# sadit/Jchemo.jl

Measured on AMD Instinct MI355X. Metric: latent-variables/sec (plskern n=1e6 p=500 q=10 nlv=25), higher is better.
Workload: dtype f64

## Files before the change

### jchemo.jl_amd/csrc/bf16.hip

```cpp
#include <stdlib.h>

#include <algorithm>
#include <type_traits>

#include "jch_internal.h"

typedef double v4f64 __attribute__((ext_vector_type(4)));
typedef unsigned short bf16_t;
typedef unsigned int v4u32 __attribute__((ext_vector_type(4)));

__device__ __forceinline__ float bf2f(bf16_t h) { return __uint_as_float(((unsigned)h) << 16); }
__device__ __forceinline__ float bflo(unsigned w) { return __uint_as_float(w << 16); }
__device__ __forceinline__ float bfhi(unsigned w) { return __uint_as_float(w & 0xffff0000u); }

template <bool VAR>
__global__ __launch_bounds__(256) void k_moments_bf16(const bf16_t *__restrict__ Xc, int64_t ldx, const bf16_t *__restrict__ Yc,
                                                       int64_t ldy, const double *__restrict__ d, int64_t n, int p, int q,
                                                       int64_t chunk, const double *__restrict__ means,
                                                       double *__restrict__ colpart)
{
    __shared__ double sc[4];
    const int j = blockIdx.x;
    const bf16_t *col = j < p ? Xc + (size_t)j * (size_t)ldx : Yc + (size_t)(j - p) * (size_t)ldy;
    const int64_t i0 = (int64_t)blockIdx.y * chunk;
// ... 594 lines not shown
        for (; b < nbx; b += 4) s0 += Kpart[(size_t)b * stride + e];
    }
    sc[g][el] = (s0 + s1) + (s2 + s3);
    __syncthreads();
    if (g == 0 && e < p * qpad) K[e] = (sc[0][el] + sc[1][el]) + (sc[2][el] + sc[3][el]);
}

template <int R>
__device__ __forceinline__ void wave_sum_rows(float (&s)[R], float (&t)[R])
{
    static_assert(R == 2 || R == 4 || R == 8, "R");
    const int lane = threadIdx.x & 63;
    float cur[R];
#pragma unroll
    for (int i = 0; i < R; ++i) cur[i] = s[i];
    int width = R;
    int bit = 32;
#pragma unroll
    for (int st = 0; st < 3; ++st) {
        if (width > 1) {
            const int half = width / 2;
            const bool hi = (lane & bit) != 0;
#pragma unroll
            for (int i = 0; i < R / 2; ++i) {
                if (i < half) {
                    const float mine = hi ? cur[half + i] : cur[i];
                    const float other = hi ? cur[i] : cur[half + i];
                    cur[i] = mine + __shfl_xor(other, bit, 64);
                }
            }
            width = half;
            bit >>= 1;
        }
    }
    float c = cur[0];
    for (int o = bit; o > 0; o >>= 1) c += __shfl_xor(c, o, 64);
#pragma unroll
    for (int r = 0; r < R; ++r) {
        int src = 0;
        if (R == 8) src = ((r >> 2) & 1) * 32 + ((r >> 1) & 1) * 16 + (r & 1) * 8;
        if (R == 4) src = ((r >> 1) & 1) * 32 + (r & 1) * 16;
        if (R == 2) src = (r & 1) * 32;
        t[r] = __int_as_float(__builtin_amdgcn_readlane(__float_as_int(c), src));
    }
}

template <int KC, int R>
__global__ __launch_bounds__(256) void k_sweep_bf16(const bf16_t *__restrict__ Xr, int64_t n, int ldr, const double *__restrict__ dw,
                                                    const double *__restrict__ rvec, const double *__restrict__ mom,
                                                    const double *__restrict__ scl, int p,
                                                    double *__restrict__ tcol, double *__restrict__ part, int ldpart)
{
    extern __shared__ __attribute__((aligned(16))) double red[];
    const int lane = threadIdx.x & 63, wv = threadIdx.x >> 6;
    float rf[KC][8], zp[KC][8];
    bool in[KC];
#pragma unroll
    for (int k = 0; k < KC; ++k) {
        const int col = 8 * lane + 512 * k;
        in[k] = col < ldr;
#pragma unroll
        for (int e = 0; e < 8; ++e) { rf[k][e] = 0.f; zp[k][e] = 0.f; }
    }
    double tt = 0.0, st = 0.0;
    const int64_t ngroups = (n + R - 1) / R;
    const int64_t gstride = (int64_t)gridDim.x * 4;
    v4u32 xn[R][KC];
    double dwn[R];
    auto fetch = [&](int64_t gg) {
        const int64_t r0 = gg * R;
#pragma unroll
        for (int rr = 0; rr < R; ++rr) {
            const bool live = r0 + rr < n;
            const v4u32 *rp = reinterpret_cast<const v4u32 *>(Xr + (size_t)(r0 + rr) * (size_t)ldr) + lane;
#pragma unroll
            for (int k = 0; k < KC; ++k) xn[rr][k] = (live && in[k]) ? __builtin_nontemporal_load(rp + 64 * k) : v4u32{0u, 0u, 0u, 0u};
            dwn[rr] = live ? dw[r0 + rr] : 0.0;
        }
    };
    int64_t g = (int64_t)blockIdx.x * 4 + wv;
    if (g < ngroups) fetch(g);
    double offd = 0.0;
#pragma unroll
    for (int k = 0; k < KC; ++k) {
        const int col = 8 * lane + 512 * k;
#pragma unroll
        for (int e = 0; e < 8; ++e)
            if (col + e < p) {
                const float v = (float)(rvec[col + e] / scl[col + e]);
                rf[k][e] = v;
                offd += mom[col + e] * (double)v;
            }
    }
    const float off = (float)jch_wave_sum(offd);
    for (; g < ngroups; g += gstride) {
        const int64_t row0 = g * R;
        v4u32 x[R][KC];
        double dwc[R];
#pragma unroll
        for (int rr = 0; rr < R; ++rr) {
            dwc[rr] = dwn[rr];
#pragma unroll
            for (int k = 0; k < KC; ++k) x[rr][k] = xn[rr][k];
        }
        if (g + gstride < ngroups) fetch(g + gstride);
        double tsel = 0.0;
        float sp[R], tr[R];
#pragma unroll
        for (int rr = 0; rr < R; ++rr) {
            float s = 0.f;
#pragma unroll
            for (int k = 0; k < KC; ++k)
#pragma unroll
                for (int e = 0; e < 4; ++e) s += bflo(x[rr][k][e]) * rf[k][2 * e] + bfhi(x[rr][k][e]) * rf[k][2 * e + 1];
            sp[rr] = s;
        }
        wave_sum_rows<R>(sp, tr);
#pragma unroll
        for (int rr = 0; rr < R; ++rr) {
            const bool live = row0 + rr < n;
            const float t = tr[rr] - off;
            const float dtf = live ? (float)dwc[rr] * t : 0.f;
            tt += (double)dtf * (double)t;
            st += (double)dtf;
#pragma unroll
            for (int k = 0; k < KC; ++k)
#pragma unroll
                for (int e = 0; e < 4; ++e) {
                    zp[k][2 * e] += dtf * bflo(x[rr][k][e]);
                    zp[k][2 * e + 1] += dtf * bfhi(x[rr][k][e]);
                }
            if (lane == rr) tsel = (double)t;
        }
        if (lane < R && row0 + lane < n) tcol[row0 + lane] = tsel;
    }
    double *zred = red;
    double *tred = red + 4 * KC * 512;
#pragma unroll
    for (int k = 0; k < KC; ++k)
#pragma unroll
        for (int e = 0; e < 8; ++e) zred[wv * (KC * 512) + 8 * lane + 512 * k + e] = (double)zp[k][e];
    if (lane == 0) { tred[wv] = tt; tred[4 + wv] = st; }
    __syncthreads();
    double *prow = part + (size_t)blockIdx.x * ldpart;
    for (int c = threadIdx.x; c < ldr; c += 256)
        prow[c] = ((zred[c] + zred[KC * 512 + c]) + zred[2 * KC * 512 + c]) + zred[3 * KC * 512 + c];
    if (threadIdx.x == 0) {
        prow[ldr] = ((tred[0] + tred[1]) + tred[2]) + tred[3];
        prow[ldr + 1] = ((tred[4] + tred[5]) + tred[6]) + tred[7];
    }
}

typedef unsigned v2u32b __attribute__((ext_vector_type(2)));
__device__ __forceinline__ void bf_fold32(float &a, float b)
{
    const v2u32b r = __builtin_amdgcn_permlane32_swap(__float_as_uint(a), __float_as_uint(b), false, false);
    a = __uint_as_float(r.x) + __uint_as_float(r.y);
}
__device__ __forceinline__ void bf_fold16(float &a, float b)
{
    const v2u32b r = __builtin_amdgcn_permlane16_swap(__float_as_uint(a), __float_as_uint(b), false, false);
    a = __uint_as_float(r.x) + __uint_as_float(r.y);
}
template <int CTRL>
__device__ __forceinline__ float bf_dpp(float v)
{
    return __int_as_float(__builtin_amdgcn_update_dpp(0, __float_as_int(v), CTRL, 0xf, 0xf, true));
}
template <int R>
__device__ __forceinline__ float bf_rowsums(float (&s)[R], int lane)
{
    static_assert(R == 4 || R == 8, "R");
#pragma unroll
    for (int i = 0; i < R; i += 2) bf_fold32(s[i], s[i + 1]);
#pragma unroll
    for (int i = 0; i < R; i += 4) bf_fold16(s[i], s[i + 2]);
    float h;
    if (R == 8) {
        const bool up = (lane & 8) != 0;
        const float w = up ? s[4] : s[0], z = up ? s[0] : s[4];
        h = w + bf_dpp<0x128>(z);
    } else {
        h = s[0] + bf_dpp<0x128>(s[0]);
    }
    h += bf_dpp<0x141>(h);
    h += bf_dpp<0xB1>(h);
    h += bf_dpp<0x4E>(h);
    return h;
}
template <int R>
__device__ __forceinline__ constexpr int bf_rowsum_lane(int rr)
{
    return 16 * (((rr & 3) == 1) ? 2 : ((rr & 3) == 2) ? 1 : (rr & 3)) + (R == 8 ? 8 * (rr >> 2) : 0);
}

template <int KC, int R, bool TSTAGE = false>
__global__ __launch_bounds__(256) void k_sweep_bf16_v2(const bf16_t *__restrict__ Xr, int64_t n, int ldr, const double *__restrict__ dw,
                                                       const double *__restrict__ rvec, const double *__restrict__ mom,
                                                       const double *__restrict__ scl, int p,
                                                       double *__restrict__ tcol, double *__restrict__ part, int ldpart, int tcap = 0)
{
    extern __shared__ __attribute__((aligned(16))) double red[];
    const int lane = threadIdx.x & 63, wv = threadIdx.x >> 6;
    int coff[KC];
#pragma unroll
    for (int k = 0; k < KC; ++k) {
        const int col = 8 * lane + 512 * k;
        coff[k] = col < ldr ? col : ldr - 8;
    }
    const int64_t ngroups = (n + R - 1) / R;
    const int64_t gstride = (int64_t)gridDim.x * 4;
    constexpr int NBUF = 2;
    v4u32 X[NBUF][R][KC];
    double D[NBUF][R];
    auto fetch = [&](v4u32 (&xb)[R][KC], double (&db)[R], int64_t gg) {
        const int64_t r0 = gg * R;
#pragma unroll
        for (int rr = 0; rr < R; ++rr) {
            const int64_t row = r0 + rr < n ? r0 + rr : n - 1;
            const bf16_t *rp = Xr + (size_t)row * (size_t)ldr;
#pragma unroll
            for (int k = 0; k < KC; ++k) xb[rr][k] = __builtin_nontemporal_load(reinterpret_cast<const v4u32 *>(rp + coff[k]));
            db[rr] = dw[row];
        }
    };
    int64_t g = (int64_t)blockIdx.x * 4 + wv;
#pragma unroll
    for (int b = 0; b < NBUF - 1; ++b)
        if (g + b * gstride < ngroups) fetch(X[b], D[b], g + b * gstride);
    float rf[KC][8], zp[KC][8];
    double offd = 0.0;
#pragma unroll
    for (int k = 0; k < KC; ++k) {
        const int col = 8 * lane + 512 * k;
#pragma unroll
        for (int e = 0; e < 8; ++e) {
            rf[k][e] = 0.f; zp[k][e] = 0.f;
            if (col + e < p) {
                const float v = (float)(rvec[col + e] / scl[col + e]);
                rf[k][e] = v;
                offd += mom[col + e] * (double)v;
            }
        }
    }
    const float off = (float)jch_wave_sum(offd);
    double tt = 0.0, st = 0.0;
    double *tring = red + 4 * KC * 512 + 8 + (TSTAGE ? __builtin_amdgcn_readfirstlane(wv) * tcap * R : 0);
    int tfill = 0;
    int64_t tdone = 0;
    auto tflush = [&] {
        const int nf = __builtin_amdgcn_readfirstlane(tfill);
        const int64_t gfirst = (int64_t)blockIdx.x * 4 + wv;
        __builtin_amdgcn_fence(__ATOMIC_ACQ_REL, "wavefront");
        for (int s = 0; s < nf; s += 64 / R) {
            const int slot = s + lane / R;
            if (slot < nf) {
                const int64_t row = (gfirst + (tdone + slot) * gstride) * R + lane % R;
                const double v = tring[s * R + lane];
                if (row < n) tcol[row] = v;
            }
        }
        __builtin_amdgcn_fence(__ATOMIC_ACQ_REL, "wavefront");
        tdone += nf;
        tfill = 0;
    };
    auto process = [&](v4u32 (&x)[R][KC], double (&dv)[R], int64_t gg) {
        const int64_t row0 = gg * R;
        float sp[R];
#pragma unroll
        for (int rr = 0; rr < R; ++rr) {
            float a = 0.f;
#pragma unroll
            for (int k = 0; k < KC; ++k)
#pragma unroll
                for (int e = 0; e < 4; ++e) a += bflo(x[rr][k][e]) * rf[k][2 * e] + bfhi(x[rr][k][e]) * rf[k][2 * e + 1];
            sp[rr] = a;
        }
        const float h = bf_rowsums<R>(sp, lane) - off;
        float ttg = 0.f, stg = 0.f;
#pragma unroll
        for (int rr = 0; rr < R; ++rr) {
            const float t = __int_as_float(__builtin_amdgcn_readlane(__float_as_int(h), bf_rowsum_lane<R>(rr)));
            const float dtf = row0 + rr < n ? (float)dv[rr] * t : 0.f;
            ttg += dtf * t;
            stg += dtf;
#pragma unroll
            for (int k = 0; k < KC; ++k)
#pragma unroll
                for (int e = 0; e < 4; ++e) {
                    zp[k][2 * e] += dtf * bflo(x[rr][k][e]);
                    zp[k][2 * e + 1] += dtf * bfhi(x[rr][k][e]);
                }
        }
        tt += (double)ttg;
        st += (double)stg;
        {
            const int src = 16 * (((lane & 3) == 1) ? 2 : ((lane & 3) == 2) ? 1 : (lane & 3)) + (R == 8 ? 8 * ((lane >> 2) & 1) : 0);
            const float tl = __shfl(h, src, 64);
            if constexpr (TSTAGE) {
                if (lane < R) tring[tfill * R + lane] = (double)tl;
                if (__builtin_amdgcn_readfirstlane(++tfill) == tcap) tflush();
            } else {
                if (lane < R && row0 + lane < n) tcol[row0 + lane] = (double)tl;
            }
        }
    };
    while (g < ngroups) {
#pragma unroll
        for (int b = 0; b < NBUF; ++b) {
            if (g < ngroups) {
                const int64_t ahead = g + (NBUF - 1) * gstride;
                if (ahead < ngroups) fetch(X[(b + NBUF - 1) % NBUF], D[(b + NBUF - 1) % NBUF], ahead);
                process(X[b], D[b], g);
                g += gstride;
            }
        }
    }
    if constexpr (TSTAGE) tflush();
    double *zred = red;
    double *tred = red + 4 * KC * 512;
#pragma unroll
    for (int k = 0; k < KC; ++k)
#pragma unroll
        for (int e = 0; e < 8; ++e) zred[wv * (KC * 512) + 8 * lane + 512 * k + e] = (double)zp[k][e];
    if (lane == 0) { tred[wv] = tt; tred[4 + wv] = st; }
    __syncthreads();
    double *prow = part + (size_t)blockIdx.x * ldpart;
    for (int c = threadIdx.x; c < ldr; c += 256)
        prow[c] = ((zred[c] + zred[KC * 512 + c]) + zred[2 * KC * 512 + c]) + zred[3 * KC * 512 + c];
    if (threadIdx.x == 0) {
        prow[ldr] = ((tred[0] + tred[1]) + tred[2]) + tred[3];
        prow[ldr + 1] = ((tred[4] + tred[5]) + tred[6]) + tred[7];
    }
}

__global__ __launch_bounds__(256) void k_bf16_fix_zt(const double *__restrict__ zt, int nslice, int ldzb, int ldr_b, int p, int ldr_small,
                                                     const double *__restrict__ mom, const double *__restrict__ scl,
                                                     double *__restrict__ zt_small)
{
    const int j = blockIdx.x * 256 + threadIdx.x;
    double tt = 0.0, st = 0.0, z = 0.0;
    for (int sl = 0; sl < nslice; ++sl) {
        tt += zt[(size_t)sl * ldzb + ldr_b];
        st += zt[(size_t)sl * ldzb + ldr_b + 1];
        if (j < p) z += zt[(size_t)sl * ldzb + j];
    }
    if (j < ldr_small) zt_small[j] = j < p ? (z - mom[j] * st) / scl[j] : 0.0;
    if (j == 0) zt_small[ldr_small] = tt;
}

template <int KC, int R>
static int32_t launch_sweep_bf16_t(jch_ctx *ctx, const bf16_t *Xr, int64_t n, int ldr_b, const double *d, const double *rvec,
                                   const double *mom, const double *scl, int p, double *tcol, double *zt8, int ldzb, int *nslice)
{
    const size_t lds = sizeof(double) * (4 * KC * 512 + 8);
    static int bpc = 0;
    static jch_per_device_once occ_once;
    if (!occ_once.done(ctx->device)) {
        int nblk = 0;
        hipError_t e = hipOccupancyMaxActiveBlocksPerMultiprocessor(&nblk, k_sweep_bf16<KC, R>, 256, lds);
        bpc = (e == hipSuccess && nblk > 0) ? nblk : 2;
        if (lds > 64 * 1024)
            JCH_HIP(ctx, hipFuncSetAttribute((const void *)k_sweep_bf16<KC, R>, hipFuncAttributeMaxDynamicSharedMemorySize, 160 * 1024));
        occ_once.mark(ctx->device);
    }
    const int64_t ngroups = (n + R - 1) / R;
    const int nb = (int)std::max<int64_t>(1, std::min<int64_t>((ngroups + 3) / 4, (int64_t)ctx->cus * bpc));
    const int m = ldr_b + 2, ldpart = (m + 7) & ~7;
    JCH_TRY(jch_reserve(ctx, ctx->part, sizeof(double) * (size_t)nb * ldpart));
    double *part = (double *)ctx->part.ptr;
    (void)jch_ev(ctx);
    hipLaunchKernelGGL((k_sweep_bf16<KC, R>), dim3(nb), dim3(256), lds, ctx->stream, Xr, n, ldr_b, d, rvec, mom, scl, p, tcol, part, ldpart);
    (void)jch_ev(ctx);
    JCH_TRY(jch_launch_reduce_part8(ctx, part, nb, ldpart, m, zt8, ldzb, nslice));
    JCH_HIP(ctx, hipGetLastError());
    return JCH_OK;
}

template <int KC, int R>
static int32_t launch_sweep_bf16_v2_t(jch_ctx *ctx, const bf16_t *Xr, int64_t n, int ldr_b, const double *d, const double *rvec,
                                      const double *mom, const double *scl, int p, double *tcol, double *zt8, int ldzb, int *nslice,
                                      jch_part_view *pv = nullptr )
{
    const size_t lds0 = sizeof(double) * (4 * KC * 512 + 8);
    static_assert(sizeof(double) * (4 * KC * 512 + 8) < 64 * 1024, "the combine area and a score ring share 64 KB");
    constexpr int TCAP_MAX = (int)((64 * 1024 - sizeof(double) * (4 * KC * 512 + 8)) / (sizeof(double) * 4 * R));
    const int tstage = ctx->sweep_tstage;
    const bool staged = tstage > 0 || (tstage < 0 && jch_sweep_bf16_tstage_default(n, ctx->cus));
    static int bpc2[2] = {0, 0};
    static jch_per_device_once occ_once;
    if (!occ_once.done(ctx->device)) {
        int nblk = 0;
        hipError_t e = hipOccupancyMaxActiveBlocksPerMultiprocessor(&nblk, k_sweep_bf16_v2<KC, R>, 256, lds0);
        bpc2[0] = (e == hipSuccess && nblk > 0) ? nblk : 2;
        e = hipOccupancyMaxActiveBlocksPerMultiprocessor(&nblk, k_sweep_bf16_v2<KC, R, true>, 256, lds0 + sizeof(double) * 4 * TCAP_MAX * R);
        bpc2[1] = (e == hipSuccess && nblk > 0) ? nblk : 2;
        occ_once.mark(ctx->device);
    }
    const int bpc = bpc2[staged];
    const int64_t ngroups = (n + R - 1) / R;
    const int nb = (int)std::max<int64_t>(1, std::min<int64_t>((ngroups + 3) / 4, (int64_t)ctx->cus * bpc));
    const int m = ldr_b + 2, ldpart = (m + 7) & ~7;
    JCH_TRY(jch_reserve(ctx, ctx->part, sizeof(double) * (size_t)nb * ldpart));
    double *part = (double *)ctx->part.ptr;
    int tcap = 0;
    if (staged) tcap = (int)std::max<int64_t>(1, std::min<int64_t>(std::min(tstage > 0 ? tstage : TCAP_MAX, TCAP_MAX), (ngroups + (int64_t)nb * 4 - 1) / ((int64_t)nb * 4)));
    const size_t lds = lds0 + sizeof(double) * 4 * (size_t)tcap * R;
    const bool timed = jch_prof_sample(ctx);
    if (timed) (void)jch_ev(ctx);
    if (tcap > 0)
        hipLaunchKernelGGL((k_sweep_bf16_v2<KC, R, true>), dim3(nb), dim3(256), lds, ctx->stream, Xr, n, ldr_b, d, rvec, mom, scl, p, tcol, part, ldpart, tcap);
    else
        hipLaunchKernelGGL((k_sweep_bf16_v2<KC, R>), dim3(nb), dim3(256), lds, ctx->stream, Xr, n, ldr_b, d, rvec, mom, scl, p, tcol, part, ldpart, 0);
    if (timed) (void)jch_ev(ctx);
    if (pv) { pv->part = part; pv->nb = nb; pv->ldpart = ldpart; *nslice = 1; JCH_HIP(ctx, hipGetLastError()); return JCH_OK; }
    JCH_TRY(jch_launch_reduce_part8(ctx, part, nb, ldpart, m, zt8, ldzb, nslice));
    JCH_HIP(ctx, hipGetLastError());
    return JCH_OK;
}

__global__ __launch_bounds__(256) void k_pivot_rows_bf16(const bf16_t *__restrict__ Xc, int64_t ldx, int64_t n, int p,
                                                         const double *__restrict__ hdr, double *__restrict__ pivot)
{
    const int lane = threadIdx.x & 63, j = blockIdx.x * 4 + (threadIdx.x >> 6);
    if (j >= p) return;
    const int m = (int)(n < 256 ? n : 256);
    const int64_t stride = n / m;
    double s = 0.0;
    for (int i = lane; i < m; i += 64) s += (double)bf2f(Xc[(size_t)i * (size_t)stride + (size_t)j * (size_t)ldx]);
    s = jch_wave_sum(s);
    if (lane == 0) pivot[j] = s / m * ((double)n / hdr[1]);
}
__global__ __launch_bounds__(256) void k_extract_means_b(double *__restrict__ K, int qpad, int p, int col, const double *__restrict__ pivot,
                                                         double *__restrict__ means)
{
    const int j = blockIdx.x * 256 + threadIdx.x;
    if (j < p) { means[j] = pivot[j] + K[(size_t)j * qpad + col]; K[(size_t)j * qpad + col] = 0.0; }
}

int32_t jch_fit_plskern_bf16(jch_ctx *ctx, const jch_pls_desc &d, const void *Xv, int64_t ldx, const void *Yv, int64_t ldy,
                             const double *wdev, double *dn, double *Tdev, jch_small &s, int ldr_small, int qpad, int ldz,
                             bool fast, int *nlv_out)
{
    const int64_t n = d.n;
    const int p = (int)d.p, q = (int)d.q;
    const bf16_t *Xc = (const bf16_t *)Xv, *Yc = (const bf16_t *)Yv;
    const int ldr_b = (p + 7) & ~7;
    JCH_TRY(jch_reserve_xr(ctx, sizeof(bf16_t) * (size_t)n * ldr_b));
    JCH_TRY(jch_reserve(ctx, ctx->yr, sizeof(double) * (size_t)n * qpad));
    bf16_t *Xr = (bf16_t *)ctx->xr.ptr;
    double *Yr = (double *)ctx->yr.ptr;
    const int ldzb = (ldr_b + 2 + 7) & ~7;
    JCH_TRY(jch_reserve(ctx, ctx->gemm_b, sizeof(double) * (size_t)JCH_ZT_SLICES * ldzb));
    double *zt8 = (double *)ctx->gemm_b.ptr;
    JCH_TRY(jch_launch_weights(ctx, wdev, n, dn, s.hdr));
    int64_t n_total = n;
    if (ctx->nranks > 1 && n < std::min<int64_t>(p, d.nlv)) {
        double hdr_h[2];
        JCH_HIP(ctx, hipMemcpyAsync(hdr_h, s.hdr, sizeof hdr_h, hipMemcpyDeviceToHost, ctx->stream));
        JCH_HIP(ctx, hipStreamSynchronize(ctx->stream));
        n_total = (int64_t)(hdr_h[1] + 0.5);
    }
    const int nlv = (int)std::min<int64_t>(std::min<int64_t>(n_total, p), d.nlv);
    const bool raw_b = !d.scal && q <= 15 && ldx % 8 == 0 && ((uintptr_t)Xc) % 16 == 0 && !jch_knob_set("JCH_CENTRED_COPY");
    if (raw_b) {
        hipLaunchKernelGGL(k_pivot_rows_bf16, dim3((p + 3) / 4), dim3(256), 0, ctx->stream, Xc, ldx, n, p, s.hdr, s.scl);
        JCH_TRY(jch_allreduce_f64(ctx, s.scl, (size_t)p));
        JCH_TRY(launch_moments_bf16(ctx, Yc, ldy, Yc, ldy, dn, n, q, 0, nullptr, s.scl + p));
    } else {
    JCH_TRY(launch_moments_bf16(ctx, Xc, ldx, Yc, ldy, dn, n, p, q, nullptr, s.mom));
    if (d.scal) JCH_TRY(launch_moments_bf16(ctx, Xc, ldx, Yc, ldy, dn, n, p, q, s.mom, s.scl));
    else hipLaunchKernelGGL(k_fill_b, dim3((p + q + 255) / 256), dim3(256), 0, ctx->stream, s.scl, p + q, 1.0);
    }
    bool m32 = false;
    {
        const int ptiles = (ldr_b + 63) / 64, kp_rows = ptiles * 64, ygroups = qpad / 16;
        const int64_t nchunks = (n + 63) / 64;
        int nbx = std::max(1, (ctx->cus * 3 + ptiles * ygroups - 1) / (ptiles * ygroups));
        if (nbx > nchunks) nbx = (int)std::max<int64_t>(nchunks, 1);
        JCH_TRY(jch_reserve(ctx, ctx->kpart, sizeof(double) * (size_t)nbx * kp_rows * qpad));
        double *Kpart = (double *)ctx->kpart.ptr;
        dim3 grid(nbx, ptiles, ygroups);
        const bool v8 = ldx % 8 == 0 && ((uintptr_t)Xc) % 16 == 0;
        const int k2panel = jch_knob("JCH_BF16_K2_PANEL", 1);
        const int NHv = jch_knob("JCH_BF16_K2_NH", 2) == 4 ? 4 : 2, THv = 32 * NHv;
        const int64_t nfull = (n / THv) * THv;
        const bool panel_ok = k2panel && v8 && qpad == 16 && ldy % 8 == 0 && ((uintptr_t)Yc) % 16 == 0 && ((uintptr_t)dn) % 16 == 0;
        const bool panel = panel_ok && nfull > 0;
        m32 = panel_ok && raw_b && !wdev && jch_knob("JCH_BF16_K2_M32", 1) != 0 && NHv == 2 && (nfull > 0 || ctx->nranks > 1);
        if (m32) {
            const int ncg = (ldr_b + 511) / 512;
            const int wmax = std::min(ldr_b, 512), ntile = (wmax + 63) / 64;
            const int NTv = ntile <= 1 ? 1 : (ntile <= 2 ? 2 : (ntile <= 4 ? 4 : 8));
            const int bpc = 2;
            int G = std::max(1, ctx->cus * bpc / ncg);
            G = (int)std::min<int64_t>(G, nfull / THv);
            const int kpr = ncg * 512;
            const bool tail = nfull < n;
            JCH_TRY(jch_reserve(ctx, ctx->kpart, sizeof(double) * (size_t)(G + 1) * kpr * 16));
            Kpart = (double *)ctx->kpart.ptr;
            const size_t lds = sizeof(bf16_t) * (size_t)THv * 516 + 16;
#define JCH_K2M(NT) do { \
                static jch_per_device_once once_; \
                if (!once_.done(ctx->device)) { JCH_HIP(ctx, hipFuncSetAttribute((const void *)k_xty_bf16_panel_m32<NT, 2>, hipFuncAttributeMaxDynamicSharedMemorySize, 160 * 1024)); once_.mark(ctx->device); } \
                hipLaunchKernelGGL((k_xty_bf16_panel_m32<NT, 2>), dim3(G, ncg), dim3(256), lds, ctx->stream, Xc, ldx, Yc, ldy, nfull, p, q, Xr, ldr_b, Kpart, kpr); } while (0)
            if (nfull == 0) {  }
            else if (NTv == 1) JCH_K2M(1); else if (NTv == 2) JCH_K2M(2); else if (NTv == 4) JCH_K2M(4); else JCH_K2M(8);
#undef JCH_K2M
            JCH_HIP(ctx, hipGetLastError());
            if (tail)
                hipLaunchKernelGGL(k_xty_bf16_tail_m32, dim3((kpr * 16 + 255) / 256), dim3(256), 0, ctx->stream, Xc, ldx, Yc, ldy, nfull, (int)(n - nfull), p, q,
                                   Xr, ldr_b, Kpart + (size_t)G * kpr * 16, kpr);
            hipLaunchKernelGGL(k_reduce_kpart_bw, dim3((p * qpad + 63) / 64), dim3(256), 0, ctx->stream, Kpart, G + (tail ? 1 : 0), kpr, p, qpad, s.K);
        } else
        if (panel) {
            const int ncg = (ldr_b + 511) / 512;
            const int wmax = std::min(ldr_b, 512), ntile = (wmax + 63) / 64;
            const int NTv = ntile <= 1 ? 1 : (ntile <= 2 ? 2 : (ntile <= 4 ? 4 : 8));
            const int bpc = NHv == 2 ? 2 : 1;
            int G = std::max(1, ctx->cus * bpc / ncg);
            G = (int)std::min<int64_t>(G, nfull / THv);
            const int kpr = ncg * 512;
            const bool tail = nfull < n;
            JCH_TRY(jch_reserve(ctx, ctx->kpart, sizeof(double) * (size_t)(G + 1) * kpr * 16));
            Kpart = (double *)ctx->kpart.ptr;
            const size_t lds = sizeof(double) * (8 * NHv * 64 + (d.scal ? 1024 : 512)) + sizeof(bf16_t) * (size_t)THv * 516 + 16;
            const double *momp = raw_b ? s.scl : s.mom;
            const int onesc = raw_b ? q : -1;
#define JCH_K2PB(NT, NH, SC) do { \
                static jch_per_device_once once_; \
                if (!once_.done(ctx->device)) { JCH_HIP(ctx, hipFuncSetAttribute((const void *)k_center_xty_bf16_panel<NT, NH, SC>, hipFuncAttributeMaxDynamicSharedMemorySize, 160 * 1024)); once_.mark(ctx->device); } \
                hipLaunchKernelGGL((k_center_xty_bf16_panel<NT, NH, SC>), dim3(G, ncg), dim3(256), lds, ctx->stream, Xc, ldx, Yc, ldy, dn, nfull, p, q, momp, s.scl, \
                                   Xr, ldr_b, Yr, Kpart, kpr, onesc); } while (0)
#define JCH_K2PB_NT(NH, SC) do { if (NTv == 1) JCH_K2PB(1, NH, SC); else if (NTv == 2) JCH_K2PB(2, NH, SC); else if (NTv == 4) JCH_K2PB(4, NH, SC); else JCH_K2PB(8, NH, SC); } while (0)
            if (NHv == 2) { if (d.scal) JCH_K2PB_NT(2, true); else JCH_K2PB_NT(2, false); }
            else { if (d.scal) JCH_K2PB_NT(4, true); else JCH_K2PB_NT(4, false); }
#undef JCH_K2PB_NT
#undef JCH_K2PB
            JCH_HIP(ctx, hipGetLastError());
            if (tail) {
                const int64_t nt = n - nfull;
// ... 63 lines not shown
```

### jchemo.jl_amd/csrc/jch_internal.h

```cpp
#pragma once
#include <hip/hip_runtime.h>
#include <stdint.h>
#include <stdio.h>
#include <string.h>

#include <functional>
#include <string>
#include <vector>

#include "jchemo_hip.h"

#define JCH_MAXQ 64
#define JCH_ZT_SLICES 8
#define JCH_SWEEP_MAXP 2048

struct xcopy_key {
    const void *X; int64_t n, ldx; int p, host;
    bool operator==(const xcopy_key &o) const { return X == o.X && n == o.n && ldx == o.ldx && p == o.p && host == o.host; }
};
struct jch_buf {
    void *ptr = nullptr;
    size_t bytes = 0;
};

struct jch_uid {
    char internal[128];
};
struct jch_rccl {
    void *handle = nullptr;
    int (*GetUniqueId)(void *) = nullptr;
    int (*CommInitRank)(void **, int, jch_uid, int) = nullptr;
    int (*AllReduce)(const void *, void *, size_t, int, int, void *, hipStream_t) = nullptr;
    int (*CommDestroy)(void *) = nullptr;
    const char *(*GetErrorString)(int) = nullptr;
};

#define JCH_P2P_MAXR 16
struct jch_p2p {
    bool ready = false, tested = false;
    int nranks = 0, rank = 0;
    void *local = nullptr;
    void *peer[JCH_P2P_MAXR] = {};
    bool opened[JCH_P2P_MAXR] = {};
    unsigned long long *host_status = nullptr, *host_status_dev = nullptr;
    unsigned long long epoch = 0;
    long long timeout_ticks = 0;
    size_t cap = 0;
    unsigned long long *stats = nullptr;
};

constexpr int JCH_INFINITY_CACHE_MIB = 256;
constexpr int JCH_RESIDENT_DEFAULT_MIB = 128;
inline bool jch_sweep_tstage_default(int kc, int64_t n, int cus) { return kc == 4 && n >= (int64_t)3900 * cus; }
inline bool jch_sweep_bf16_tstage_default(int64_t n, int cus) { (void)n; (void)cus; return false; }

struct jch_ctx {
    int device = 0;
    int cus = 256;
    hipStream_t stream = nullptr;
    bool own_stream = false;
    std::string err;
    void *comm = nullptr;
    int rank = 0, nranks = 1;
    void *loop = nullptr;
    jch_p2p p2p;
    std::vector<double> loop_sum;
    void *hstage = nullptr;
    size_t hstage_bytes = 0;
    xcopy_key xcopy{};
    bool xcopy_valid = false;
    long long xcopy_reused = 0;
    unsigned sweep_seq = 0;
    int sweep_alt = 0;
    bool sweep_fused_reduce = false;
    int sweep_resident_mb = -1;
    int sweep_tstage = -1;
    jch_buf gram, xr, yr, xstage, ystage, wstage, tbuf, dnorm, part, kpart, small, colpart, gemm_b, gemm_out, xq, tickets, qz, lw_work, lw_xrm, lvws, lw_flags, lw_screen;
    jch_buf kg_ws, dk_x, dk_y, dk_k, dk_q, dk_o, dk_s;
    jch_buf kp_ws;
    jch_buf kc_vt, pc_ws, pc_vec;
    jch_buf chol_inv, chol_a, chol_w, chol_s, kr_ws;
    jch_buf rp_stage, rp_rows, rp_coef;
    jch_buf cs_ws, cs_part;
    jch_buf xt_part, xt_ws;
    jch_buf sel_ws, sel_out;
    jch_buf st_t, st_ms;
    jch_buf sp_ws;
    jch_buf kn_ws;
    jch_buf kd_ws;
    jch_buf gd_ws;
    const void *chol_L = nullptr;
    int64_t chol_n = 0, chol_ld = 0;
    bool profiling = false;
    int prof_stride = 1;
    unsigned prof_seq = 0;
    int64_t sweeps_timed = 0;
    jch_profile prof{};
    std::vector<hipEvent_t> ev_pool;
    size_t ev_used = 0;
    size_t ev_mark = 0;
    std::vector<hipEvent_t> cev_pool;
    std::vector<int> cev_phase;
    size_t cev_used = 0;
    int coll_phase = 0;
    bool coll_in_fit = false;
    int coll_transport = 0;
    hipStream_t aux_stream = nullptr;
    hipEvent_t aux_event = nullptr;
    long long pivot_refits = 0;
    long long knn_screened = 0, knn_screen_redone = 0;
    long long locw_refits = 0;
};

struct jch_per_device_once {
    unsigned long long mask = 0;
    bool done(int dev) const { return (mask >> (dev & 63)) & 1ull; }
    void mark(int dev) { mask |= 1ull << (dev & 63); }
};

struct jch_carve {
    size_t off = 0;
    size_t take(size_t count) { const size_t o = off; off += (count + 31) & ~(size_t)31; return o; }
};

int32_t jch_fail(jch_ctx *ctx, int32_t code, const char *fmt, ...);
#define JCH_HIP(ctx, expr)                                                                         \
    do {                                                                                           \
        hipError_t e__ = (expr);                                                                   \
        if (e__ != hipSuccess)                                                                     \
            return jch_fail(ctx, e__ == hipErrorOutOfMemory ? JCH_ENOMEM : JCH_EHIP, "%s: %s (%s:%d)", #expr, \
                            hipGetErrorString(e__), __FILE__, __LINE__);                           \
    } while (0)
#define JCH_TRY(expr)                 \
    do {                              \
        int32_t s__ = (expr);         \
        if (s__ != JCH_OK) return s__; \
    } while (0)

bool jch_knob_set(const char *name);
int jch_knob(const char *name, int dflt);

int32_t jch_reserve(jch_ctx *ctx, jch_buf &b, size_t bytes);
inline int32_t jch_reserve_xstage(jch_ctx *ctx, size_t bytes, bool keep_copy = false) {
    if (!keep_copy && ctx->xcopy.host) ctx->xcopy_valid = false;
    return jch_reserve(ctx, ctx->xstage, bytes);
}
inline int32_t jch_reserve_xr(jch_ctx *ctx, size_t bytes, bool keep_copy = false) {
    if (!keep_copy) ctx->xcopy_valid = false;
    return jch_reserve(ctx, ctx->xr, bytes);
}
int32_t jch_reserve_host(jch_ctx *ctx, size_t bytes);
int32_t jch_allreduce_f64(jch_ctx *ctx, double *dev_buf, size_t count);
int32_t jch_allreduce_slices(jch_ctx *ctx, double *zt, int m, int nslice, int ldz, int *nslice_out);
int32_t jch_p2p_allreduce(jch_ctx *ctx, const double *src, size_t count, int nslice, int ldz, double *dst);
int32_t jch_p2p_check(jch_ctx *ctx);
void jch_p2p_destroy(jch_ctx *ctx);

struct jch_span {
    hipEvent_t a = nullptr, b = nullptr;
};
hipEvent_t jch_ev(jch_ctx *ctx);
bool jch_prof_sample(jch_ctx *ctx);
void jch_coll_begin(jch_ctx *ctx);
void jch_coll_end(jch_ctx *ctx);
void jch_coll_reset(jch_ctx *ctx);
void jch_coll_collect(jch_ctx *ctx, jch_profile &pr);

struct jch_part_view {
    const double *part = nullptr;
    int nb = 0, ldpart = 0;
};

int32_t jch_launch_weights(jch_ctx *ctx, const double *w_dev , int64_t n, double *dnorm,
                           double *hdr , double *zero0 = nullptr, int nzero0 = 0,
                           double *zero1 = nullptr, int nzero1 = 0 );
int32_t jch_launch_moments(jch_ctx *ctx, const double *Xc, int64_t ldx, const double *Yc, int64_t ldy,
                           const double *d, int64_t n, int p, int q, const double *means ,
                           double *out , bool do_sqrt = true);
int32_t jch_launch_center_xty(jch_ctx *ctx, double *Xc, int64_t ldx, double *Yc, int64_t ldy, const double *d,
                              int64_t n, int p, int q, const double *mom, const double *scl, bool writeback,
                              double *Xr, int ldr, double *Yr, int qpad, double *K , bool scal,
                              double *means_out = nullptr ,
                              double *mshift_out = nullptr ,
                              const double *spread2 = nullptr ,
                              double *qual = nullptr ,
                              double *ones_out = nullptr );
int32_t jch_launch_pivot(jch_ctx *ctx, const double *Xc, int64_t ldx, int64_t n, int p, const double *hdr ,
                         double *pivot , double *spread2 );
int32_t jch_launch_export_colmajor(jch_ctx *ctx, const double *Xr, int ldr, const double *Yr, int qpad, int64_t n,
                                   int p, int q, double *Xc, int64_t ldx, double *Yc, int64_t ldy,
                                   const double *sqrt_rowscale = nullptr );
int32_t jch_launch_sweep(jch_ctx *ctx, const double *Xr, int64_t n, int p, int ldr, const double *d, const double *rvec,
                         const double *Yr, int qpad, int q_extra ,
                         double *tcol, double *zt , int ldz, int max_slices,
                         int *nslice_out, const double *mu = nullptr ,
                         jch_part_view *pv = nullptr );
int32_t jch_launch_reduce_rows(jch_ctx *ctx, const double *part, int nb, int ldpart, int m, double *out);
int32_t jch_launch_xty_rows(jch_ctx *ctx, const double *Xr, int ldr, const double *Yc, int64_t ldy, const double *d, int64_t n, int p, int q,
                            const double *mom, double *Yr, int qpad, double *K, double *means_out, double *mshift_out,
                            const double *spread2, double *qual, double *ones_out, bool *done);
int32_t jch_launch_raw_scales(jch_ctx *ctx, const double *Xr, int64_t n, int p, int ldr, const double *d, const double *mshift,
                              const double *Yr, int qpad, int q, double *tmp, double *scl, double *K);
int32_t jch_launch_reduce_part8(jch_ctx *ctx, const double *part, int nb, int ldpart, int m, double *zt, int ldz, int *nslice_out);
int32_t jch_launch_sweep_wide(jch_ctx *ctx, const double *Xr, int64_t n, int ldr, const double *d, const double *rvec,
                              const double *Yr, int qpad, bool nipals, double *tcol, double *zt);
int32_t jch_launch_ytdt(jch_ctx *ctx, const double *Yr, int64_t n, int qpad, const double *d, const double *tcol, double *out );
#define JCH_NIPALS_DEFER_DEFAULT 6
// ... 145 lines not shown
```

Before: 1540.

## Rework bf16 sweep kernel addressing, packed FMA math, and score staging defaults

Rewrites the bf16 sweep kernel's inner loops. Row addressing now goes through scalar base pointers with unsigned vector offsets, and each lane loads a single row weight instead of R of them. Dot products and z accumulation use packed two-wide float FMAs, and for KC>1 the bf16 values are re-widened rather than kept live, to reduce register pressure. Score writes drop the shuffle and use the 8-lane-group row mapping, launch bounds gain a minimum-blocks hint, and score staging is now on by default for KC==1 at large n. This lowers VALU and register cost per row in exchange for more complex indexing and new occupancy constraints.

```diff
diff --git a/jchemo.jl_amd/csrc/bf16.hip b/jchemo.jl_amd/csrc/bf16.hip
--- a/jchemo.jl_amd/csrc/bf16.hip
+++ b/jchemo.jl_amd/csrc/bf16.hip
@@ -770,6 +770,9 @@
 }
 
 typedef unsigned v2u32b __attribute__((ext_vector_type(2)));
+typedef float v2f32b __attribute__((ext_vector_type(2)));
+typedef __attribute__((address_space(1))) v4u32 bf_gv4u32;
+typedef __attribute__((address_space(1))) double bf_gf64;
 __device__ __forceinline__ void bf_fold32(float &a, float b)
 {
     const v2u32b r = __builtin_amdgcn_permlane32_swap(__float_as_uint(a), __float_as_uint(b), false, false);
@@ -813,50 +816,66 @@
 }
 
 template <int KC, int R, bool TSTAGE = false>
-__global__ __launch_bounds__(256) void k_sweep_bf16_v2(const bf16_t *__restrict__ Xr, int64_t n, int ldr, const double *__restrict__ dw,
+__global__ __launch_bounds__(256, (KC > 1 && TSTAGE) ? 1 : 2) void k_sweep_bf16_v2(const bf16_t *__restrict__ Xr, int64_t n, int ldr, const double *__restrict__ dw,
                                                        const double *__restrict__ rvec, const double *__restrict__ mom,
                                                        const double *__restrict__ scl, int p,
                                                        double *__restrict__ tcol, double *__restrict__ part, int ldpart, int tcap = 0)
 {
+    static_assert(R == 8, "one weight per 8-lane group of the row sums");
     extern __shared__ __attribute__((aligned(16))) double red[];
-    const int lane = threadIdx.x & 63, wv = threadIdx.x >> 6;
-    int coff[KC];
+    const int lane = threadIdx.x & 63, wv = __builtin_amdgcn_readfirstlane((int)(threadIdx.x >> 6));
+    unsigned coff[KC];
 #pragma unroll
     for (int k = 0; k < KC; ++k) {
         const int col = 8 * lane + 512 * k;
-        coff[k] = col < ldr ? col : ldr - 8;
-    }
+        coff[k] = 2u * (unsigned)(col < ldr ? col : ldr - 8);
+    }
+    const unsigned myrow = (unsigned)((((lane >> 4) & 1) << 1) | ((lane >> 5) & 1) | (((lane >> 3) & 1) << 2));
     const int64_t ngroups = (n + R - 1) / R;
     const int64_t gstride = (int64_t)gridDim.x * 4;
+    const size_t rowbytes = sizeof(bf16_t) * (size_t)ldr;
     constexpr int NBUF = 2;
+    constexpr bool REWIDEN = KC > 1;
     v4u32 X[NBUF][R][KC];
-    double D[NBUF][R];
-    auto fetch = [&](v4u32 (&xb)[R][KC], double (&db)[R], int64_t gg) {
+    double D[NBUF];
+    auto fetch = [&](v4u32 (&xb)[R][KC], double &db, int64_t gg) {
         const int64_t r0 = gg * R;
+        const int64_t left = n - 1 - r0;
+        const unsigned last = left < R - 1 ? (unsigned)left : (unsigned)(R - 1);
+        const char *rp = reinterpret_cast<const char *>(Xr) + (size_t)r0 * rowbytes;
+        unsigned cl[KC];
+#pragma unroll
+        for (int k = 0; k < KC; ++k) {
+            cl[k] = coff[k];
+            asm("" : "+v"(cl[k]));
+        }
 #pragma unroll
         for (int rr = 0; rr < R; ++rr) {
-            const int64_t row = r0 + rr < n ? r0 + rr : n - 1;
-            const bf16_t *rp = Xr + (size_t)row * (size_t)ldr;
-#pragma unroll
-            for (int k = 0; k < KC; ++k) xb[rr][k] = __builtin_nontemporal_load(reinterpret_cast<const v4u32 *>(rp + coff[k]));
-            db[rr] = dw[row];
-        }
+            if (rr > 0) rp += (unsigned)rr <= last ? rowbytes : 0;
+            uint64_t rb = reinterpret_cast<uint64_t>(rp);
+            asm("" : "+s"(rb));
+#pragma unroll
+            for (int k = 0; k < KC; ++k) xb[rr][k] = __builtin_nontemporal_load(reinterpret_cast<const bf_gv4u32 *>(rb + cl[k]));
+        }
+        uint64_t db0 = reinterpret_cast<uint64_t>(dw + r0);
+        asm("" : "+s"(db0));
+        db = *reinterpret_cast<const bf_gf64 *>(db0 + sizeof(double) * (myrow < last ? myrow : last));
     };
     int64_t g = (int64_t)blockIdx.x * 4 + wv;
 #pragma unroll
     for (int b = 0; b < NBUF - 1; ++b)
         if (g + b * gstride < ngroups) fetch(X[b], D[b], g + b * gstride);
-    float rf[KC][8], zp[KC][8];
+    v2f32b rf[KC][4], zp[KC][4];
     double offd = 0.0;
 #pragma unroll
     for (int k = 0; k < KC; ++k) {
         const int col = 8 * lane + 512 * k;
 #pragma unroll
         for (int e = 0; e < 8; ++e) {
-            rf[k][e] = 0.f; zp[k][e] = 0.f;
+            rf[k][e >> 1][e & 1] = 0.f; zp[k][e >> 1][e & 1] = 0.f;
             if (col + e < p) {
                 const float v = (float)(rvec[col + e] / scl[col + e]);
-                rf[k][e] = v;
+                rf[k][e >> 1][e & 1] = v;
                 offd += mom[col + e] * (double)v;
             }
         }
@@ -882,45 +901,54 @@
         tdone += nf;
         tfill = 0;
     };
-    auto process = [&](v4u32 (&x)[R][KC], double (&dv)[R], int64_t gg) {
+    auto process = [&](v4u32 (&x)[R][KC], double dv, int64_t gg) {
         const int64_t row0 = gg * R;
+        const int64_t left = n - row0;
+        const bool live = left >= R || myrow < (unsigned)left;
+        v2f32b xf[R][KC][4];
         float sp[R];
 #pragma unroll
         for (int rr = 0; rr < R; ++rr) {
-            float a = 0.f;
+            v2f32b a = {0.f, 0.f};
 #pragma unroll
             for (int k = 0; k < KC; ++k)
 #pragma unroll
-                for (int e = 0; e < 4; ++e) a += bflo(x[rr][k][e]) * rf[k][2 * e] + bfhi(x[rr][k][e]) * rf[k][2 * e + 1];
-            sp[rr] = a;
+                for (int e = 0; e < 4; ++e) {
+                    xf[rr][k][e] = v2f32b{bflo(x[rr][k][e]), bfhi(x[rr][k][e])};
+                    a = __builtin_elementwise_fma(xf[rr][k][e], rf[k][e], a);
+                }
+            sp[rr] = a.x + a.y;
         }
         const float h = bf_rowsums<R>(sp, lane) - off;
+        const float dth = live ? (float)dv * h : 0.f;
         float ttg = 0.f, stg = 0.f;
 #pragma unroll
         for (int rr = 0; rr < R; ++rr) {
             const float t = __int_as_float(__builtin_amdgcn_readlane(__float_as_int(h), bf_rowsum_lane<R>(rr)));
-            const float dtf = row0 + rr < n ? (float)dv[rr] * t : 0.f;
-            ttg += dtf * t;
+            const float dtf = __int_as_float(__builtin_amdgcn_readlane(__float_as_int(dth), bf_rowsum_lane<R>(rr)));
+            ttg = __builtin_fmaf(dtf, t, ttg);
             stg += dtf;
+            const v2f32b dt2 = {dtf, dtf};
 #pragma unroll
             for (int k = 0; k < KC; ++k)
 #pragma unroll
                 for (int e = 0; e < 4; ++e) {
-                    zp[k][2 * e] += dtf * bflo(x[rr][k][e]);
-                    zp[k][2 * e + 1] += dtf * bfhi(x[rr][k][e]);
+                    v2f32b xv = xf[rr][k][e];
+                    if constexpr (REWIDEN) {
+                        unsigned w = x[rr][k][e];
+                        asm("" : "+v"(w));
+                        xv = v2f32b{bflo(w), bfhi(w)};
+                    }
+                    zp[k][e] = __builtin_elementwise_fma(dt2, xv, zp[k][e]);
                 }
         }
         tt += (double)ttg;
         st += (double)stg;
-        {
-            const int src = 16 * (((lane & 3) == 1) ? 2 : ((lane & 3) == 2) ? 1 : (lane & 3)) + (R == 8 ? 8 * ((lane >> 2) & 1) : 0);
-            const float tl = __shfl(h, src, 64);
-            if constexpr (TSTAGE) {
-                if (lane < R) tring[tfill * R + lane] = (double)tl;
-                if (__builtin_amdgcn_readfirstlane(++tfill) == tcap) tflush();
-            } else {
-                if (lane < R && row0 + lane < n) tcol[row0 + lane] = (double)tl;
-            }
+        if constexpr (TSTAGE) {
+            if ((lane & 7) == 0) tring[tfill * R + myrow] = (double)h;
+            if (__builtin_amdgcn_readfirstlane(++tfill) == tcap) tflush();
+        } else {
+            if ((lane & 7) == 0 && live) tcol[row0 + myrow] = (double)h;
         }
     };
     while (g < ngroups) {
@@ -940,7 +968,7 @@
 #pragma unroll
     for (int k = 0; k < KC; ++k)
 #pragma unroll
-        for (int e = 0; e < 8; ++e) zred[wv * (KC * 512) + 8 * lane + 512 * k + e] = (double)zp[k][e];
+        for (int e = 0; e < 8; ++e) zred[wv * (KC * 512) + 8 * lane + 512 * k + e] = (double)zp[k][e >> 1][e & 1];
     if (lane == 0) { tred[wv] = tt; tred[4 + wv] = st; }
     __syncthreads();
     double *prow = part + (size_t)blockIdx.x * ldpart;
@@ -1004,7 +1032,7 @@
     static_assert(sizeof(double) * (4 * KC * 512 + 8) < 64 * 1024, "the combine area and a score ring share 64 KB");
     constexpr int TCAP_MAX = (int)((64 * 1024 - sizeof(double) * (4 * KC * 512 + 8)) / (sizeof(double) * 4 * R));
     const int tstage = ctx->sweep_tstage;
-    const bool staged = tstage > 0 || (tstage < 0 && jch_sweep_bf16_tstage_default(n, ctx->cus));
+    const bool staged = tstage > 0 || (tstage < 0 && jch_sweep_bf16_tstage_default(KC, n, ctx->cus));
     static int bpc2[2] = {0, 0};
     static jch_per_device_once occ_once;
     if (!occ_once.done(ctx->device)) {
diff --git a/jchemo.jl_amd/csrc/jch_internal.h b/jchemo.jl_amd/csrc/jch_internal.h
--- a/jchemo.jl_amd/csrc/jch_internal.h
+++ b/jchemo.jl_amd/csrc/jch_internal.h
@@ -52,7 +52,7 @@
 constexpr int JCH_INFINITY_CACHE_MIB = 256;
 constexpr int JCH_RESIDENT_DEFAULT_MIB = 128;
 inline bool jch_sweep_tstage_default(int kc, int64_t n, int cus) { return kc == 4 && n >= (int64_t)3900 * cus; }
-inline bool jch_sweep_bf16_tstage_default(int64_t n, int cus) { (void)n; (void)cus; return false; }
+inline bool jch_sweep_bf16_tstage_default(int kc, int64_t n, int cus) { return kc == 1 && n >= (int64_t)3900 * cus; }
 
 struct jch_ctx {
     int device = 0;
```

Result: no change. 1539 (-0.1%).
